# WoodOxen/tactics2d

Hardware: NVIDIA H100
Metric: participant_steps_per_sec (higher is better)
Workload: dtype f32

## Files before the change

### tactics2d_b200/csrc/t2d_kernels.cu

```cuda
#include <cuda_runtime.h>
#include <stddef.h>
#include <stdint.h>
#include <stdio.h>
#include <string.h>

#include <algorithm>
#include <atomic>
#include <cmath>
#include <memory>
#include <mutex>
#include <string>
#include <vector>

#include "../../include/t2d_b200.h"
#include "t2d_math.cuh"

namespace t2d {

constexpr int MAX_WARPS_PER_CTA = 8;
constexpr int CTA_THREADS = MAX_WARPS_PER_CTA * 32;
constexpr int PPL = 4;
constexpr int POSE_PER_WARP = 32 * PPL;
constexpr int MAP_SMEM_LIMIT = 120 * 1024;

struct MapHeader {
  int32_t n_seg, gx, gy, n_items;
  float x0, y0, inv_cell, cell;
  uint32_t off_seg, off_cell, off_items, total_bytes;
  uint32_t off_clear;
  int32_t fine;
  uint32_t off_dcell, off_ditems;
  float dil;
  int32_t n_ditems;
  uint32_t off_objfirst;
  int32_t n_poly;
  uint32_t off_poly;
  uint32_t off_pbox;
  uint32_t off_fine;
  uint32_t smem_bytes;
  float bxmin, bxmax, bymin, bymax;
  int32_t has_bounds;
  uint32_t pad[3];
};
constexpr float CLEAR_QUANT = 0.125f;
static_assert(sizeof(MapHeader) == 128, "MapHeader must be 128 bytes");

struct WorldArgs {
  float *x, *y, *h, *v, *vx, *vy;
  const uint8_t* type_id;
  int32_t* step_count;
  const Params* table;
  int n_types, N, M;
};

struct MapArgs {
  const unsigned char* map_blob;
  const uint32_t* tile_off;
  const uint16_t* tile_id;
};

__device__ __forceinline__ const unsigned char* tile_blob(const MapArgs& m, long long n) {
  return m.map_blob ? m.map_blob + (m.tile_id ? m.tile_off[m.tile_id[n]] : 0u) : nullptr;
}

struct GoalArgs {
  const float* target;
  float* iou;
  float* last_pose;
  int32_t* noact_count;
  float threshold;
  int noact_max;
};

struct StepArgs {
  float *x, *y, *h, *v, *vx, *vy;
  const uint8_t* type_id;
  int32_t* step_count;
  const float* action;
  const float* ego_action;
  uint8_t* flags;
  int16_t* hit_index;
  int16_t* hit_segment;
  uint8_t* scn_status;
  uint8_t* done;
  const unsigned char* map_blob;
  const uint32_t* tile_off;
  const uint16_t* tile_id;
  MapHeader mh;
  const Params* table;
  int map_bytes, map_in_smem;
  int n_types;
  int N, M, G;
  int g_shift, mp_shift, unused1, n_tiles, wpc, table_bytes;
  int off_poseA, off_poseB, off_hit, off_queue, off_sorted, unused0, off_qcount, off_bar;
  int n_steps;
  float dt, dt_rem;
  double dt_d, dt_rem_d, interval_d;
  int max_step, cfg_flags;
  int do_physics, has_bounds, vec_ok, needs_vel_in;
  int prefetch;
  float bxmin, bxmax, bymin, bymax;
  float rb_max;
  GoalArgs goal;
  float *wheel_f, *wheel_r;
};

__device__ __forceinline__ uint32_t smem_u32(const void* p) { return (uint32_t)__cvta_generic_to_shared(p); }

__device__ __forceinline__ void mbar_init(uint64_t* bar, uint32_t count) {
  asm volatile("mbarrier.init.shared::cta.b64 [%0], %1;" ::"r"(smem_u32(bar)), "r"(count));
}
__device__ __forceinline__ void fence_mbar_init() { asm volatile("fence.mbarrier_init.release.cluster;" ::: "memory"); }
__device__ __forceinline__ void mbar_expect_tx(uint64_t* bar, uint32_t bytes) {
  asm volatile("mbarrier.arrive.expect_tx.shared::cta.b64 _, [%0], %1;" ::"r"(smem_u32(bar)), "r"(bytes) : "memory");
}
__device__ __forceinline__ void bulk_g2s(void* dst, const void* src, uint32_t bytes, uint64_t* bar) {
  asm volatile("cp.async.bulk.shared::cluster.global.mbarrier::complete_tx::bytes [%0], [%1], %2, [%3];" ::"r"(
                   smem_u32(dst)),
               "l"(src), "r"(bytes), "r"(smem_u32(bar))
               : "memory");
}
__device__ __forceinline__ void mbar_wait(uint64_t* bar, uint32_t parity) {
  uint32_t ok = 0;
  while (!ok) {
    asm volatile(
        "{\n\t.reg .pred p;\n\t"
        "mbarrier.try_wait.parity.shared::cta.b64 p, [%1], %2;\n\t"
        "selp.u32 %0, 1, 0, p;\n\t}"
        : "=r"(ok)
        : "r"(smem_u32(bar)), "r"(parity)
        : "memory");
  }
}

template <int BYTES> struct VecOf;
template <> struct VecOf<1> { using T = uint8_t; };
template <> struct VecOf<2> { using T = uint16_t; };
template <> struct VecOf<4> { using T = uint32_t; };
template <> struct VecOf<8> { using T = uint2; };
template <> struct VecOf<16> { using T = uint4; };

template <typename T, int N>
__device__ __forceinline__ void ld_vec(const T* p, T (&o)[N]) {
  using V = typename VecOf<sizeof(T) * N>::T;
  const V v = *reinterpret_cast<const V*>(p);
  memcpy(o, &v, sizeof(V));
}
template <typename T, int N>
__device__ __forceinline__ void st_vec(T* p, const T (&o)[N]) {
  using V = typename VecOf<sizeof(T) * N>::T;
  V v;
  memcpy(&v, o, sizeof(V));
  *reinterpret_cast<V*>(p) = v;
}

struct Pose {
  float x, y, h, c, s, l, w;
};

__device__ __noinline__ bool pair_exact(const Pose a, const Pose b) {
  const bool ca = a.w < 0.0f, cb = b.w < 0.0f;
  if (!ca && !cb) return obb_obb_f64(a.x, a.y, a.h, a.l, a.w, b.x, b.y, b.h, b.l, b.w);
  if (!ca && cb) return obb_circle_f64(a.x, a.y, a.h, a.l, a.w, b.x, b.y, b.l);
  if (ca && !cb) return obb_circle_f64(b.x, b.y, b.h, b.l, b.w, a.x, a.y, a.l);
  return circle_circle_f64(a.x, a.y, a.l, b.x, b.y, b.l);
}

__device__ __forceinline__ bool pair_hit(const Pose& a, const Pose& b) {
  const bool ca = a.w < 0.0f, cb = b.w < 0.0f;
  int r;
  if (!ca && !cb) r = obb_obb_f32(a.x, a.y, a.c, a.s, a.l, a.w, b.x, b.y, b.c, b.s, b.l, b.w);
  else if (!ca && cb) r = obb_circle_f32(a.x, a.y, a.c, a.s, a.l, a.w, b.x, b.y, b.l);
  else if (ca && !cb) r = obb_circle_f32(b.x, b.y, b.c, b.s, b.l, b.w, a.x, a.y, a.l);
  else r = circle_circle_f32(a.x, a.y, a.l, b.x, b.y, b.l);
  if (r < 0) return pair_exact(a, b);
  return r != 0;
}

__device__ __noinline__ bool seg_exact(const Pose a, const float4 sg) {
  if (a.w < 0.0f) return circle_segment_f64(a.x, a.y, a.l, sg.x, sg.y, sg.z, sg.w);
  return obb_segment_f64(a.x, a.y, a.h, a.l, a.w, sg.x, sg.y, sg.z, sg.w);
}

__device__ __forceinline__ bool seg_hit(const Pose& a, const float4 sg) {
  int r = a.w < 0.0f ? circle_segment_f32(a.x, a.y, a.l, sg.x, sg.y, sg.z, sg.w)
                     : obb_segment_f32(a.x, a.y, a.c, a.s, a.l, a.w, sg.x, sg.y, sg.z, sg.w);
  if (r < 0) return seg_exact(a, sg);
// ... 409 lines not shown
    if (nvalid == PPL && K1_SHAPE(vec_ok, 1)) {
      ld_vec<float, PPL>(A.x + idx0, sx);
      ld_vec<float, PPL>(A.y + idx0, sy);
      ld_vec<float, PPL>(A.h + idx0, shd);
      ld_vec<float, PPL>(A.v + idx0, sv);
      uint8_t tb8[PPL];
      ld_vec<uint8_t, PPL>(A.type_id + idx0, tb8);
#pragma unroll
      for (int i = 0; i < PPL; ++i) tidv[i] = tb8[i];
      if (K1_SHAPE(do_physics, 1)) {
        float2 act[PPL];
        float lo[4], hi[4];
        ld_vec<float, 4>(A.action + 2 * idx0, lo);
        ld_vec<float, 4>(A.action + 2 * idx0 + 4, hi);
        act[0] = make_float2(lo[0], lo[1]); act[1] = make_float2(lo[2], lo[3]);
        act[2] = make_float2(hi[0], hi[1]); act[3] = make_float2(hi[2], hi[3]);
#pragma unroll
        for (int i = 0; i < PPL; ++i) { a0[i] = act[i].x; a1[i] = act[i].y; }
        if (K1_SHAPE(needs_vel_in, 0)) {
          ld_vec<float, PPL>(A.vx + idx0, svx);
          ld_vec<float, PPL>(A.vy + idx0, svy);
        }
      }
    } else {
#pragma unroll
      for (int i = 0; i < PPL; ++i) {
        if (i < nvalid) {
          sx[i] = A.x[idx0 + i]; sy[i] = A.y[idx0 + i]; shd[i] = A.h[idx0 + i]; sv[i] = A.v[idx0 + i];
          tidv[i] = A.type_id[idx0 + i];
          if (K1_SHAPE(do_physics, 1)) {
            a0[i] = A.action[2 * (idx0 + i)]; a1[i] = A.action[2 * (idx0 + i) + 1];
            if (K1_SHAPE(needs_vel_in, 0)) { svx[i] = A.vx[idx0 + i]; svy[i] = A.vy[idx0 + i]; }
          }
        }
      }
    }
    if (cohorts && !cohort_b && tile == tile0) cohort_arrive(wpc * 32);
    {
      const long long n_next = n + (long long)gridDim.x * wpc * spw;
      if (A.prefetch && n_next < A.N && m0 < M) prefetch_tile_l2<FIXED>(A, n_next * M + m0);
    }
    if (K1_SHAPE(ego_action, nullptr) != nullptr && K1_SHAPE(do_physics, 1) && gl == 0 && scn_ok) {
      const float2 ea = reinterpret_cast<const float2*>(K1_SHAPE(ego_action, nullptr))[n];
      a0[0] = ea.x; a1[0] = ea.y;
    }
    if (!staged) {
      mbar_wait(s_bar, 0);
      staged = true;
    }
    float ch[PPL], sh[PPL];
    bool active[PPL], kin[PPL];
    const Params* pp[PPL];
    int model[PPL];
    bool lane_all_kin = true, lane_any_kin = false;
#pragma unroll
    for (int i = 0; i < PPL; ++i) {
      active[i] = tidv[i] < A.n_types;
      pp[i] = &s_table[active[i] ? tidv[i] : 0];
      model[i] = pp[i]->model_shape & 0xff;
      kin[i] = active[i] && (model[i] == MODEL_KINEMATICS);
      lane_all_kin = lane_all_kin && kin[i];
      lane_any_kin = lane_any_kin || kin[i];
      ch[i] = 1.0f; sh[i] = 0.0f;
    }
    T2D_TL(2, tl_on, tl_slot, sx[PPL - 1] + sy[PPL - 1] + shd[PPL - 1] + sv[PPL - 1] + a0[PPL - 1] + a1[PPL - 1] + (float)model[PPL - 1]);
    if (A.cfg_flags & T2D_CFG_STEER_FIRST) {
#pragma unroll
      for (int i = 0; i < PPL; ++i)
        if (model[i] <= MODEL_DYNAMICS || model[i] == MODEL_DRIFT) { float t = a0[i]; a0[i] = a1[i]; a1[i] = t; }
    }

    if (K1_SHAPE(do_physics, 1)) {
      if (__any_sync(0xffffffffu, lane_any_kin)) {
        const Params* const null_row = &s_table[A.n_types];
        const Params* pk[PPL];
        KinIO<PPL> io;
#pragma unroll
        for (int i = 0; i < PPL; ++i) {
          pk[i] = kin[i] ? pp[i] : null_row;
          io.x[i] = kin[i] ? sx[i] : 0.0f; io.y[i] = kin[i] ? sy[i] : 0.0f;
          io.h[i] = kin[i] ? shd[i] : 0.0f; io.v[i] = kin[i] ? sv[i] : 0.0f;
          io.acc[i] = kin[i] ? a0[i] : 0.0f; io.steer[i] = kin[i] ? a1[i] : 0.0f;
        }
        kinematics_step<PPL>(io, pk, A.n_steps, A.dt, A.dt_rem);
#pragma unroll
        for (int i = 0; i < PPL; ++i) {
          if (kin[i]) {
            sx[i] = io.x[i]; sy[i] = io.y[i]; shd[i] = io.h[i]; sv[i] = io.v[i];
            svx[i] = io.vx[i]; svy[i] = io.vy[i]; ch[i] = io.ch[i]; sh[i] = io.sh[i];
          }
        }
      }
      if (!lane_all_kin) {
#pragma unroll
        for (int i = 0; i < PPL; ++i) {
          if (active[i] && !kin[i]) {
            if constexpr (!KIN_ONLY) {
              OneIO io;
              io.x = sx[i]; io.y = sy[i]; io.h = shd[i]; io.v = sv[i]; io.vx = svx[i]; io.vy = svy[i];
              io.a0 = a0[i]; io.a1 = a1[i];
              io.ch = 1.0f; io.sh = 0.0f;
              other_model_step(io, *pp[i], A.n_steps, A.dt_d, A.dt_rem_d, A.interval_d);
              sx[i] = io.x; sy[i] = io.y; shd[i] = io.h; sv[i] = io.v; svx[i] = io.vx; svy[i] = io.vy;
              ch[i] = io.ch; sh[i] = io.sh;
            } else {
              sincos_fast(shd[i], &sh[i], &ch[i]);
            }
          }
        }
      }
      bool all_active = true;
#pragma unroll
      for (int i = 0; i < PPL; ++i) all_active = all_active && active[i];
      if (nvalid == PPL && K1_SHAPE(vec_ok, 1) && all_active) {
        st_vec<float, PPL>(A.x + idx0, sx);
        st_vec<float, PPL>(A.y + idx0, sy);
        st_vec<float, PPL>(A.h + idx0, shd);
        st_vec<float, PPL>(A.v + idx0, sv);
        st_vec<float, PPL>(A.vx + idx0, svx);
        st_vec<float, PPL>(A.vy + idx0, svy);
      } else {
#pragma unroll
        for (int i = 0; i < PPL; ++i) {
          if (i < nvalid && active[i]) {
            A.x[idx0 + i] = sx[i]; A.y[idx0 + i] = sy[i]; A.h[idx0 + i] = shd[i]; A.v[idx0 + i] = sv[i];
            A.vx[idx0 + i] = svx[i]; A.vy[idx0 + i] = svy[i];
          }
        }
      }
    } else {
#pragma unroll
      for (int i = 0; i < PPL; ++i) sincos_fast(shd[i], &sh[i], &ch[i]);
    }
    T2D_TL(3, tl_on, tl_slot, sx[0] + sy[PPL - 1] + ch[0] + sh[PPL - 1]);

    float px[PPL], py[PPL], rb[PPL];
    unsigned solid_bits = 0;
#pragma unroll
    for (int i = 0; i < PPL; ++i) {
      const Vec4 g2 = params_group(pp[i], 2);
      const bool sol = active[i] && (__float_as_int(g2.w) >> 8) != SHAPE_NONE;
      solid_bits |= sol ? (1u << i) : 0u;
      rb[i] = g2.z;
      px[i] = sol ? sx[i] : __int_as_float(0x7fc00000);
      py[i] = sy[i];
      poseA[i * 32 + lane] = make_float4(px[i], py[i], rb[i], shd[i]);
      poseB[i * 32 + lane] = make_float4(ch[i], sh[i], g2.x, g2.y);
    }
    if (lane == 0) *qcount = 0;
    __syncwarp();
    const int cnt_in = (K1_SHAPE(do_physics, 1) && gl == 0 && scn_ok) ? A.step_count[n] : 0;

    unsigned near_q[PPL], near_alt[PPL];
#pragma unroll
    for (int i = 0; i < PPL; ++i) { near_q[i] = 255u; near_alt[i] = 255u; }
    const MapHeader* lane_mh = &A.mh;
    const unsigned char* lane_blob = A.map_blob;
    if constexpr (MAP_TABLE) {
      lane_blob = A.map_blob + A.tile_off[scn_ok ? A.tile_id[n] : 0];
      lane_mh = reinterpret_cast<const MapHeader*>(lane_blob);
    }
    if (A.map_blob != nullptr && lane_mh->n_seg > 0) {
#pragma unroll
      for (int i = 0; i < PPL; ++i) {
        unsigned alt;
        near_q[i] = near_fetch(px[i], py[i], rb[i], *lane_mh, lane_blob + lane_mh->off_fine, alt);
        near_alt[i] = ((solid_bits >> i) & 1u) ? alt : 255u;
// ... 667 lines not shown
  const long long total = (long long)A.N * A.M;
  for (long long i = (long long)blockIdx.x * blockDim.x + threadIdx.x; i < total; i += (long long)gridDim.x * blockDim.x) {
    const int n = (int)(i / A.M), m = (int)(i - (long long)n * A.M);
    int row;
    if (A.mask != nullptr) {
      if (!A.mask[n]) continue;
      row = A.pool_index ? A.pool_index[n] : n;
      row = min(max(row, 0), A.n_rows - 1);
      if (m == 0) A.log_row_out[n] = row;
    } else {
      row = min(max(A.log_row[n], 0), A.n_rows - 1);
    }
    const long long s = (long long)row * A.M + m;
    int k;
    long long t;
    if (A.slot_track1 != nullptr) {
      k = __ldg(A.slot_track1 + s);
      if (k < 0) {
        if (A.track_out) A.track_out[i] = -1;
        continue;
      }
      t = (long long)A.t0[row] + ((long long)A.step_count[n] + A.offset) * A.interval_ms;
    } else {
      int lo = __ldg(A.slot_off + s), hi = __ldg(A.slot_off + s + 1) - 1;
      if (hi < lo) {
        if (A.track_out) A.track_out[i] = -1;
        continue;
      }
      t = (long long)A.t0[row] + ((long long)A.step_count[n] + A.offset) * A.interval_ms;
      while (lo < hi) {
        const int mid = (lo + hi) >> 1;
        if ((long long)__ldg(&A.entries[mid].last_ms) >= t) hi = mid;
        else lo = mid + 1;
      }
      k = __ldg(&A.entries[lo].track);
    }
    const int4 tr4 = __ldg(reinterpret_cast<const int4*>(A.tracks) + k);
    const int first = tr4.x, period = tr4.y, n_frames = tr4.z, rec_off = tr4.w;
    const long long d = t - first;
    if (d < 0 || d > (long long)(n_frames - 1) * period) {
      A.type_id[i] = T2D_TYPE_INACTIVE;
      if (A.track_out) A.track_out[i] = -1;
      continue;
    }
    if (A.track_out) A.track_out[i] = k;
    const long long j = d / period;
    const int r = (int)(d - j * period);
    const float* a = A.rec + 5 * ((long long)rec_off + j);
    float x, y, h, vx, vy;
    if (r == 0) {
      x = a[0]; y = a[1]; h = a[2]; vx = a[3]; vy = a[4];
    } else {
      const float* b = a + 5;
      const double w = __ddiv_rn((double)r, (double)period);
      x = replay_lerp(a[0], b[0], w);
      y = replay_lerp(a[1], b[1], w);
      vx = replay_lerp(a[3], b[3], w);
      vy = replay_lerp(a[4], b[4], w);
      const double ha = (double)a[2];
      double dh = __dsub_rn((double)b[2], ha);
      if (dh > PI_D) dh = __dsub_rn(dh, TWO_PI_D);
      else if (dh < -PI_D) dh = __dadd_rn(dh, TWO_PI_D);
      double hh = __dadd_rn(ha, __dmul_rn(w, dh));
      if (hh < 0.0) hh = __dadd_rn(hh, TWO_PI_D);
      else if (hh >= TWO_PI_D) hh = __dsub_rn(hh, TWO_PI_D);
      h = __double2float_rn(hh);
      if (h == (float)TWO_PI_D) h = 0.0f;
    }
    const float v = __double2float_rn(__dsqrt_rn(__dadd_rn(__dmul_rn((double)vx, (double)vx), __dmul_rn((double)vy, (double)vy))));
    A.x[i] = x; A.y[i] = y; A.h[i] = h; A.v[i] = v; A.vx[i] = vx; A.vy[i] = vy;
    A.type_id[i] = A.track_type[k];
  }
}

struct PhysArgs {
  Params p;
  float *x, *y, *h, *v, *vx, *vy;
  float *wheel_f, *wheel_r;
  const float* action;
  float* applied;
  int n, n_steps;
  float dt, dt_rem;
  double dt_d, dt_rem_d, interval_d;
};

__global__ void __launch_bounds__(256) t2d_physics_kernel(const __grid_constant__ PhysArgs A) {
  for (long long i = (long long)blockIdx.x * blockDim.x + threadIdx.x; i < A.n; i += (long long)gridDim.x * blockDim.x) {
    if (A.p.model() == MODEL_KINEMATICS) {
      KinIO<1> io;
      io.x[0] = A.x[i]; io.y[0] = A.y[i]; io.h[0] = A.h[i]; io.v[0] = A.v[i];
      io.acc[0] = A.action[2 * i]; io.steer[0] = A.action[2 * i + 1];
      const Params* const p1[1] = {&A.p};
      kinematics_step<1>(io, p1, A.n_steps, A.dt, A.dt_rem);
      A.x[i] = io.x[0]; A.y[i] = io.y[0]; A.h[i] = io.h[0]; A.v[i] = io.v[0]; A.vx[i] = io.vx[0]; A.vy[i] = io.vy[0];
      if (A.applied) { A.applied[2 * i] = io.acc[0]; A.applied[2 * i + 1] = io.steer[0]; }
    } else {
      OneIO io;
      io.x = A.x[i]; io.y = A.y[i]; io.h = A.h[i]; io.v = A.v[i]; io.vx = A.vx[i]; io.vy = A.vy[i];
      io.a0 = A.action[2 * i]; io.a1 = A.action[2 * i + 1];
      io.ch = 1.0f; io.sh = 0.0f;
      if (A.p.model() == MODEL_DRIFT) {
        io.w0 = A.wheel_f[i]; io.w1 = A.wheel_r[i];
        drift_step(io, A.p, A.n_steps, A.dt_d, A.dt_rem_d);
        A.wheel_f[i] = io.w0; A.wheel_r[i] = io.w1;
      } else {
        other_model_step(io, A.p, A.n_steps, A.dt_d, A.dt_rem_d, A.interval_d);
      }
      A.x[i] = io.x; A.y[i] = io.y; A.h[i] = io.h; A.v[i] = io.v; A.vx[i] = io.vx; A.vy[i] = io.vy;
      if (A.applied) { A.applied[2 * i] = io.a0; A.applied[2 * i + 1] = io.a1; }
    }
  }
}

constexpr int LIDAR_EDGES = 144;
constexpr int LIDAR_WARPS = 4;
constexpr int LIDAR_BEAMS = 512;

struct LidarArgs : WorldArgs {
  MapArgs map;
  const double* beam_cs;
  const int16_t* observers;
  float* scan;
  int Q, n_beams;
  double range;
};

__device__ __forceinline__ double point_segment_dist2(double x1, double y1, double x2, double y2) {
  const double dx = x2 - x1, dy = y2 - y1, dd = dx * dx + dy * dy;
  double t = dd > 0.0 ? -(x1 * dx + y1 * dy) / dd : 0.0;
  t = fmin(fmax(t, 0.0), 1.0);
  const double ex = x1 + t * dx, ey = y1 + t * dy;
  return ex * ex + ey * ey;
}

__global__ void __launch_bounds__(LIDAR_WARPS * 32, 7) t2d_lidar_kernel(const __grid_constant__ LidarArgs A) {
  __shared__ double s_edge[LIDAR_WARPS][LIDAR_EDGES][4];
  __shared__ BeamWindow s_win[LIDAR_WARPS][LIDAR_EDGES];
  __shared__ float s_best[LIDAR_WARPS][LIDAR_BEAMS];
  __shared__ int s_cnt[LIDAR_WARPS];
  const int lane = threadIdx.x & 31, warp = threadIdx.x >> 5;
  const long long row = (long long)blockIdx.x * LIDAR_WARPS + warp;
  if (row >= (long long)A.N * A.Q) return;
  const long long n = A.Q == 1 ? row : row <= 0xffffffffll ? (long long)((unsigned)row / (unsigned)A.Q) : row / A.Q;
  const int q = (int)(row - n * A.Q);
  const int jo = A.observers ? (int)A.observers[row] : q;
  double(*edge)[4] = s_edge[warp];
  BeamWindow* win = s_win[warp];
  float* best = s_best[warp];
  int* cnt = &s_cnt[warp];
  const long long base = n * A.M;
  float* out = A.scan + row * A.n_beams;
  if (jo < 0 || jo >= A.M || A.type_id[base + jo] >= A.n_types) {
    for (int b = lane; b < A.n_beams; b += 32) out[b] = INFINITY;
    return;
  }
  const double x0 = A.x[base + jo], y0 = A.y[base + jo], th = A.h[base + jo];
  double sa, ca;
  sincos(th, &sa, &ca);
  const double xoff = -x0 * ca - y0 * sa, yoff = x0 * sa - y0 * ca;
  const double R = A.range, R2 = R * R;
  const unsigned char* blob = tile_blob(A.map, n);
  const MapHeader* tmh = reinterpret_cast<const MapHeader*>(blob);
  const int n_seg = blob ? tmh->n_seg : 0;
  const float4* seg = n_seg > 0 ? reinterpret_cast<const float4*>(blob + tmh->off_seg) : nullptr;
  const int part_rounds = (A.M - 1 + 31) / 32, seg_rounds = (n_seg + 31) / 32;
  for (int b0 = 0; b0 < A.n_beams; b0 += LIDAR_BEAMS) {
    const int nb = min(LIDAR_BEAMS, A.n_beams - b0);
    for (int k = lane; k < nb; k += 32) best[k] = INFINITY;
    if (lane == 0) *cnt = 0;
    __syncwarp();
    for (int r = 0; r < part_rounds + seg_rounds; ++r) {
      if (r < part_rounds) {
        const int i = r * 32 + lane;
        const int j = i < jo ? i : i + 1;
        const int tj = j < A.M ? (int)A.type_id[base + j] : 255;
        if (tj < A.n_types && A.table[tj].shape() == SHAPE_OBB) {
// ... 540 lines not shown
  const uint8_t* ctrl_id = nullptr;
  const int16_t* ctrl_lead = nullptr;
  const int16_t* ctrl_path = nullptr;
  float* ctrl_last_accel = nullptr;
  bool ctrl_has_pid = false;
  bool ctrl_pid_reads_target = false;
  const float* pid_target = nullptr;
  double* pid_state = nullptr;
  dev_ptr<PathVertex> d_path_v;
  dev_ptr<int> d_path_off;
  int n_paths = 0;
  const int16_t* route_id = nullptr;
  double route_threshold = 0.0, route_weight = 0.0;
  float route_off_reward = 0.0f;
  double* route_s_best = nullptr;
  double* route_agent_s_best = nullptr;
  int route_agent_rows = 0;
  std::unique_ptr<ChunkedUpload> hs_upload;
  Mirror hs_out;
  MappedEgo hs_ego;
  AgentStaging ha;
  dev_ptr<uint8_t> ha_flags;
  int host_chunks = 0;
  int n_bev_styles = 0;
  t2d_bev_style bev_style[bev::MAX_STYLES] = {};
  uint8_t bev_type_style[T2D_MAX_TYPES] = {};
  int bev_target_style = bev::NO_STYLE;
  std::unique_ptr<DeviceLog> log;
  std::vector<int> type_model;
};

enum : unsigned { NEED_STATE = 1, NEED_TABLE = 2, NEED_TICK = 4 };

static int require(const t2d_ctx* c, unsigned need) {
  if ((need & NEED_STATE) && !c->x) return fail(T2D_E_STATE, "state not bound: call t2d_bind_state first");
  if ((need & NEED_TABLE) && (!c->d_table || c->n_types == 0))
    return fail(T2D_E_STATE, "type table not set: call t2d_set_type_table first");
  if (need & NEED_TICK) {
    if (c->has_drift && !(c->wheel_f && c->wheel_r))
      return fail(T2D_E_STATE, "the type table holds a SingleTrackDrift row: call t2d_bind_wheel_state first");
    if (c->log && c->log->type_id != c->type_id) return fail(T2D_E_STATE, "state rebound after t2d_set_log: call t2d_set_log again");
  }
  return T2D_OK;
}

static WorldArgs world_args(const t2d_ctx* c) {
  return {c->x, c->y, c->h, c->v, c->vx, c->vy, c->type_id, c->step_count, c->d_table.get(), c->n_types, c->N, c->M};
}

static RouteArgs route_args(const t2d_ctx* c) {
  return {c->route_id, c->d_path_v.get(), c->d_path_off.get(), c->n_paths, c->route_off_reward, c->route_threshold,
          c->route_weight};
}

static int check_route_trackers(const t2d_ctx* c, const char* fn) {
  if (c->route_id && c->route_agent_s_best && c->route_agent_rows != c->agent_q)
    return fail(T2D_E_STATE, std::string(fn) + ": the agents' route tracker has another row count than the bound agents: "
                                               "call t2d_bind_route_trackers again");
  return T2D_OK;
}

static MapArgs map_args(const DeviceMap& map, int first = 0) {
  return {map.blob.get(), map.tile_off.get(), map.tile_id ? map.tile_id + first : nullptr};
}

static int launched() {
  g_launches.fetch_add(1);
  CUDA_TRY(cudaGetLastError());
  return T2D_OK;
}

static int capped_grid(long long items, int per_cta, int sm_count, int per_sm) {
  return (int)std::max(1LL, std::min((items + per_cta - 1) / per_cta, (long long)sm_count * per_sm));
}

template <class Args> static void set_time_step(Args& A, int interval_ms, int delta_t_ms) {
  const int delta_t = std::min(delta_t_ms, interval_ms);
  A.n_steps = interval_ms / delta_t;
  A.dt = (float)((double)delta_t / 1000.0);
  A.dt_rem = (float)((double)(interval_ms % delta_t) / 1000.0);
  A.dt_d = (double)delta_t / 1000.0;
  A.dt_rem_d = (double)(interval_ms % delta_t) / 1000.0;
  A.interval_d = (double)interval_ms / 1000.0;
}

extern "C" {

int t2d_version(void) { return T2D_VERSION; }
const char* t2d_last_error(void) { return g_err.c_str(); }
int64_t t2d_launch_count(void) { return (int64_t)g_launches.load(); }
int64_t t2d_tick_fixed_count(void) { return (int64_t)(g_tick_instances[4].load() + g_tick_instances[5].load()); }
int64_t t2d_tick_instance_count(int k) { return k >= 0 && k < 7 ? (int64_t)g_tick_instances[k].load() : -1; }

#ifdef T2D_TICK_TIMELINE
int t2d_tick_timeline(void* dst, int64_t bytes, int clear) {
  if (!dst || bytes != (int64_t)sizeof(t2d_timeline)) return fail(T2D_E_INVALID, "timeline buffer size");
  CUDA_TRY(cudaMemcpyFromSymbol(dst, t2d_timeline, sizeof(t2d_timeline)));
  if (clear) {
    void* p = nullptr;
    CUDA_TRY(cudaGetSymbolAddress(&p, t2d_timeline));
    CUDA_TRY(cudaMemset(p, 0, sizeof(t2d_timeline)));
  }
  return T2D_OK;
}
#endif

static int check_cfg(const t2d_config* cfg) {
  if (!cfg) return fail(T2D_E_INVALID, "cfg is NULL");
  if (cfg->interval_ms <= 0) return fail(T2D_E_INVALID, "interval_ms must be > 0");
  if (cfg->delta_t_ms <= 0) return fail(T2D_E_INVALID, "delta_t_ms must be > 0");
  return T2D_OK;
}

int t2d_create(t2d_ctx** out, int device, int n_scenarios, int m_participants, const t2d_config* cfg) {
  if (!out) return fail(T2D_E_INVALID, "out is NULL");
  *out = nullptr;
  if (int r = check_cfg(cfg)) return r;
  if (n_scenarios <= 0 || m_participants <= 0) return fail(T2D_E_INVALID, "n_scenarios and m_participants must be > 0");
  if (m_participants > T2D_MAX_PARTICIPANTS)
    return fail(T2D_E_UNSUPPORTED, "m_participants > 128: a scenario must fit one warp (4 participants per lane)");
  int count = 0;
  CUDA_TRY(cudaGetDeviceCount(&count));
  if (device < 0 || device >= count) return fail(T2D_E_INVALID, "no such CUDA device");
  CUDA_TRY(cudaSetDevice(device));
  t2d_ctx* c = new t2d_ctx();
  c->device = device;
  c->N = n_scenarios;
  c->M = m_participants;
  if (const char* e = getenv("T2D_PDL")) c->use_pdl = atoi(e) != 0;
  if (const char* e = getenv("T2D_GRID_LIMIT")) c->grid_limit = std::max(0, atoi(e));
  if (const char* e = getenv("T2D_TICK_GENERIC")) c->tick_generic = atoi(e) != 0;
  if (const char* e = getenv("T2D_PREFETCH")) c->prefetch_override = atoi(e) != 0 ? 1 : 0;
  if (const char* e = getenv("T2D_WPC")) {
    const int v = atoi(e);
    if (v >= 1 && v <= MAX_WARPS_PER_CTA) c->wpc_override = v;
  }
  if (const char* e = getenv("T2D_HOST_CHUNKS")) c->host_chunks = std::max(0, std::min(atoi(e), MAX_HOST_CHUNKS));
  int g = 1;
  while (g * PPL < m_participants) g <<= 1;
  c->G = g;
  c->cfg = *cfg;
  cudaDeviceProp prop;
  CUDA_TRY(cudaGetDeviceProperties(&prop, device));
  c->sm_count = prop.multiProcessorCount;
  c->max_smem_optin = (int)prop.sharedMemPerBlockOptin;
  *out = c;
  return T2D_OK;
}

int t2d_destroy(t2d_ctx* c) {
  if (!c) return T2D_OK;
  cudaSetDevice(c->device);
  delete c;
  return T2D_OK;
}

int t2d_set_config(t2d_ctx* c, const t2d_config* cfg) {
  if (!c) return fail(T2D_E_INVALID, "ctx is NULL");
  if (int r = check_cfg(cfg)) return r;
  c->cfg = *cfg;
  return T2D_OK;
}

int t2d_set_type_table(t2d_ctx* c, const t2d_type_params* table, int n_types) {
  if (!c || !table) return fail(T2D_E_INVALID, "ctx/table is NULL");
  if (n_types <= 0 || n_types > T2D_MAX_TYPES) return fail(T2D_E_INVALID, "n_types must be in 1..64");
// ... 1303 lines not shown
```

### tactics2d_b200/csrc/t2d_math.cuh

```cuda
#pragma once

#include <math.h>
#include <string.h>
#include <stdint.h>

#if defined(__CUDACC__)
#define T2D_HD __host__ __device__ __forceinline__
#define T2D_HD_NOINLINE __host__ __device__ __noinline__
#else
#define T2D_HD inline
#define T2D_HD_NOINLINE
#endif

#if defined(__CUDA_ARCH__)
#define T2D_RSQRTF(x) rsqrtf(x)
#else
#define T2D_RSQRTF(x) (1.0f / sqrtf(x))
#endif

namespace t2d {

constexpr int MODEL_KINEMATICS = 0;
constexpr int MODEL_DYNAMICS = 1;
constexpr int MODEL_POINTMASS_NEWTON = 2;
// ... 67 lines not shown
#endif
}

#if defined(__CUDA_ARCH__)
#define T2D_FDIV(a, b) __fdividef((a), (b))
#else
#define T2D_FDIV(a, b) ((a) / (b))
#endif

constexpr float RINT_MAGIC = 12582912.0f;

T2D_HD float wrap_two_pi(float phi) {
  const float q = (fmaf(phi, INV_TWO_PI, -0.5f) + RINT_MAGIC) - RINT_MAGIC;
  float r = fmaf(-q, TWO_PI_HI, phi);
  r = fmaf(-q, TWO_PI_LO, r);
  if (r < 0.0f) r += TWO_PI_HI;
  if (r >= TWO_PI_HI) r -= TWO_PI_HI;
  if (r < 0.0f) r = 0.0f;
  return r;
}

struct SinCos { float s, c; };
#if defined(__CUDACC__)
__host__ __device__ __noinline__ SinCos sincosf_slow(float x) { SinCos r; sincosf(x, &r.s, &r.c); return r; }
#else
inline SinCos sincosf_slow(float x) { SinCos r; sincosf(x, &r.s, &r.c); return r; }
#endif

T2D_HD void sincos_poly(float r, float& s, float& c) {
  const float z = r * r;
  s = fmaf(r * z, fmaf(z, fmaf(z, -1.9515295891e-4f, 8.3321608736e-3f), -1.6666654611e-1f), r);
  c = fmaf(z * z, fmaf(z, fmaf(z, 2.443315711809948e-5f, -1.388731625493765e-3f), 4.166664568298827e-2f),
           fmaf(-0.5f, z, 1.0f));
}

T2D_HD void sincos_core(float x, float& so, float& co) {
  const float t = fmaf(x, 0.636619772f, RINT_MAGIC);
  const float k = t - RINT_MAGIC;
  float r = fmaf(-k, 1.570556640625f, x);
  r = fmaf(-k, 2.396702766418457e-4f, r);
  r = fmaf(-k, 1.5893254712295857e-8f, r);
  float s, c;
  sincos_poly(r, s, c);
  const int q = float_bits(t);
  const float a = (q & 1) ? c : s, b = (q & 1) ? s : c;
  so = (q & 2) ? -a : a;
  co = ((q + 1) & 2) ? -b : b;
}

T2D_HD void sincos_fast(float x, float* sn, float* cs) {
  float so, co;
  if (!(fabsf(x) <= 512.0f)) {
    const SinCos r = sincosf_slow(x);
    so = r.s; co = r.c;
  } else {
    sincos_core(x, so, co);
  }
  *sn = so;
  *cs = co;
}

constexpr float SIN_C3 = -1.6666667e-1f, SIN_C5 = 8.3333333e-3f;
constexpr float COS_C2 = -0.5f, COS_C4 = 4.1666667e-2f, COS_C6 = -1.3888889e-3f;

T2D_HD void rotate_small(float& c, float& s, float d, float nd) {
  const float dd = d * d;
  const float ts = fmaf(dd, fmaf(dd, SIN_C5, SIN_C3), 1.0f);
  const float sn = d * ts, nsn = nd * ts;
  const float nhv = dd * fmaf(dd, fmaf(dd, COS_C6, COS_C4), COS_C2);
  const float cn = fmaf(s, nsn, fmaf(c, nhv, c));
  const float sm = fmaf(c, sn, fmaf(s, nhv, s));
  c = cn;
  s = sm;
}

template <int W>
struct KinIO {
  float x[W], y[W], h[W], v[W];
  float vx[W], vy[W];
  float ch[W], sh[W];
  float acc[W], steer[W];
};

template <int W>
T2D_HD void kinematics_finish(KinIO<W>& io, const Params* const (&p)[W], const float (&c)[W], const float (&s)[W], float (&v)[W],
                              const float (&Sx)[W], const float (&Sy)[W], const float (&Sv)[W], const float (&kdt)[W],
                              const float (&k)[W], const float (&a)[W], const float (&vlo)[W], const float (&vhi)[W], float dt,
                              float dt_rem) {
#pragma unroll
  for (int i = 0; i < W; ++i) {
    float x = fmaf(dt, Sx[i], io.x[i]);
    float y = fmaf(dt, Sy[i], io.y[i]);
    float dphi = kdt[i] * Sv[i];
    if (dt_rem > 0.0f) {
      x = fmaf(dt_rem * v[i], c[i], x);
      y = fmaf(dt_rem * v[i], s[i], y);
      dphi = fmaf(k[i] * dt_rem, v[i], dphi);
      v[i] = clampf(fmaf(a[i], dt_rem, v[i]), vlo[i], vhi[i]);
    }
    float hn = wrap_two_pi(io.h[i] + dphi);
    float sh, ch;
    sincos_core(hn, sh, ch);
    io.x[i] = x; io.y[i] = y; io.h[i] = hn; io.v[i] = v[i];
    io.vx[i] = v[i] * ch;
    io.vy[i] = v[i] * sh;
    io.ch[i] = ch; io.sh[i] = sh;
  }
}

template <int W>
T2D_HD void kinematics_step(KinIO<W>& io, const Params* const (&p)[W], int n_steps, float dt, float dt_rem) {
  float c[W], s[W], w1[W], Sx[W], Sy[W], Sv[W], kdt[W], adt[W], vlo[W], vhi[W], k[W], a[W];
  bool small = true;
  bool lin = n_steps >= 2 && n_steps <= 24;
  float sd[W], cd[W], sp[W], cp[W];
  bool rare = false;
#pragma unroll
  for (int i = 0; i < W; ++i) {
    const Vec4 g0 = params_group(p[i], 0);
    a[i] = clampf(io.acc[i], g0.x, g0.y);
    const float d = clampf(io.steer[i], g0.z, g0.w);
    io.acc[i] = a[i];
    io.steer[i] = d;
    sincos_poly(d, sd[i], cd[i]);
    sincos_core(io.h[i], sp[i], cp[i]);
    rare = rare || !(fabsf(d) <= 0.78f) || !(fabsf(io.h[i]) <= 512.0f);
  }
  if (rare) {
#pragma unroll
    for (int i = 0; i < W; ++i) {
      if (!(fabsf(io.steer[i]) <= 0.78f)) sincos_fast(io.steer[i], &sd[i], &cd[i]);
      if (!(fabsf(io.h[i]) <= 512.0f)) sincos_fast(io.h[i], &sp[i], &cp[i]);
    }
  }
#pragma unroll
  for (int i = 0; i < W; ++i) {
    const Vec4 g1 = params_group(p[i], 1);
    const float tan_d = T2D_FDIV(sd[i], cd[i]);
    const float tb = g1.z * tan_d;
    const float cb = T2D_RSQRTF(fmaf(tb, tb, 1.0f));
    const float sb = tb * cb;
    k[i] = tan_d * cb * g1.w;
    kdt[i] = k[i] * dt;
    adt[i] = a[i] * dt;
    c[i] = cp[i] * cb - sp[i] * sb;
    s[i] = sp[i] * cb + cp[i] * sb;
    vlo[i] = g1.x;
    vhi[i] = g1.y;
    const float w1u = fmaf(a[i], dt, io.v[i]);
    w1[i] = clampf(w1u, vlo[i], vhi[i]);
    const float wlu = fmaf((float)(n_steps - 1), adt[i], w1[i]);
    const float wl = clampf(fmaf((float)(n_steps - 2), adt[i], w1[i]), vlo[i], vhi[i]);
    lin = lin && (w1u == w1[i]) && (wlu >= vlo[i]) && (wlu <= vhi[i]) && (fabsf(kdt[i] * adt[i]) <= 1e-4f);
    const float wmax = fmaxf(fabsf(io.v[i]), fmaxf(fabsf(w1[i]), fabsf(wl)));
    small = small && (fabsf(kdt[i]) * wmax <= 0.25f);
    Sx[i] = 0.0f; Sy[i] = 0.0f; Sv[i] = 0.0f;
  }
#if defined(__CUDA_ARCH__)
  const bool fast = __all_sync(__activemask(), lin && small);
#else
  const bool fast = lin && small;
#endif
  if (fast) {
    float h[W], nsn[W], se[W], nse[W], he[W];
#pragma unroll
    for (int i = 0; i < W; ++i) {
      const float d0 = kdt[i] * io.v[i], dd = d0 * d0;
      const float ts = fmaf(dd, fmaf(dd, SIN_C5, SIN_C3), 1.0f);
      nsn[i] = (-d0) * ts;
      h[i] = dd * fmaf(dd, fmaf(dd, COS_C6, COS_C4), COS_C2);
      se[i] = kdt[i] * adt[i];
      nse[i] = -se[i];
      he[i] = -0.5f * se[i] * se[i];
    }
    float v[W];
#pragma unroll
    for (int i = 0; i < W; ++i) v[i] = io.v[i];
    {
      float fi = -1.0f;
      for (int it = 0; it < n_steps; ++it) {
        fi += 1.0f;
#pragma unroll
        for (int i = 0; i < W; ++i) {
          Sx[i] = fmaf(v[i], c[i], Sx[i]);
          Sy[i] = fmaf(v[i], s[i], Sy[i]);
          const float sn = -nsn[i];
          const float cn = fmaf(s[i], nsn[i], fmaf(c[i], h[i], c[i]));
          const float sm = fmaf(c[i], sn, fmaf(s[i], h[i], s[i]));
          const float hn = fmaf(nsn[i], se[i], h[i] + he[i]);
          const float nn = fmaf(h[i], nse[i], nsn[i] + nse[i]);
          c[i] = cn; s[i] = sm; h[i] = hn; nsn[i] = nn;
          v[i] = fmaf(fi, adt[i], w1[i]);
        }
      }
    }
    const float nm1 = (float)(n_steps - 1), tri = 0.5f * (float)(n_steps - 1) * (float)(n_steps - 2);
#pragma unroll
    for (int i = 0; i < W; ++i) Sv[i] = fmaf(tri, adt[i], fmaf(nm1, w1[i], io.v[i]));
    kinematics_finish<W>(io, p, c, s, v, Sx, Sy, Sv, kdt, k, a, vlo, vhi, dt, dt_rem);
    return;
  }
  float v[W];
#pragma unroll
  for (int i = 0; i < W; ++i) v[i] = io.v[i];
  if (small) {
    float fi = -1.0f;
    for (int it = 0; it < n_steps; ++it) {
      fi += 1.0f;
#pragma unroll
      for (int i = 0; i < W; ++i) {
        Sx[i] = fmaf(v[i], c[i], Sx[i]);
        Sy[i] = fmaf(v[i], s[i], Sy[i]);
        Sv[i] += v[i];
        rotate_small(c[i], s[i], kdt[i] * v[i], -kdt[i] * v[i]);
        v[i] = clampf(fmaf(fi, adt[i], w1[i]), vlo[i], vhi[i]);
      }
    }
  } else {
    float fi = -1.0f;
    for (int it = 0; it < n_steps; ++it) {
      fi += 1.0f;
#pragma unroll
      for (int i = 0; i < W; ++i) {
        Sx[i] = fmaf(v[i], c[i], Sx[i]);
        Sy[i] = fmaf(v[i], s[i], Sy[i]);
        Sv[i] += v[i];
        float sn, cs;
        sincos_fast(kdt[i] * v[i], &sn, &cs);
        const float c2 = c[i] * cs - s[i] * sn;
        const float s2 = s[i] * cs + c[i] * sn;
        c[i] = c2;
        s[i] = s2;
        v[i] = clampf(fmaf(fi, adt[i], w1[i]), vlo[i], vhi[i]);
      }
    }
  }
  kinematics_finish<W>(io, p, c, s, v, Sx, Sy, Sv, kdt, k, a, vlo, vhi, dt, dt_rem);
}

struct OneIO {
  float x, y, h, v, vx, vy;
  float ch, sh;
  float a0, a1;
  float w0, w1;
};

template <int W>
T2D_HD void dynamics_step_n(OneIO* const (&io)[W], const Params* const (&pp)[W], int n_steps, double dt) {
  double x[W], y[W], phi[W], v[W], d_phi[W], beta[W], sn[W], cs[W];
  double accel[W], delta[W], tan_d[W], L[W], vlo[W], vhi[W], d_beta_slow[W], mu[W];
  double k_a[W], k_sum[W], k_dif[W], k_cc[W], lf_cf_f[W], cf_f[W];
#pragma unroll
  for (int i = 0; i < W; ++i) {
    const Params& p = *pp[i];
    const double lf = p.lf, lr = p.lr;
    L[i] = (double)p.lf + (double)p.lr;
    accel[i] = clampd(io[i]->a0, p.accel_lo, p.accel_hi);
    delta[i] = clampd(io[i]->a1, p.steer_lo, p.steer_hi);
    io[i]->a0 = (float)accel[i];
    io[i]->a1 = (float)delta[i];
    const double mass = p.mass, h = p.mass_height, Iz = p.I_z, cf = p.cf, cr = p.cr;
    mu[i] = p.mu;
    const double factor_f = (G_ACC * lr - accel[i] * h) / L[i];
    const double factor_r = (G_ACC * lf + accel[i] * h) / L[i];
    lf_cf_f[i] = lf * cf * factor_f;
    const double lr_cr_r = lr * cr * factor_r;
    const double lf2_cf_f = lf * lf * cf * factor_f, lr2_cr_r = lr * lr * cr * factor_r;
    cf_f[i] = cf * factor_f;
    const double cr_r = cr * factor_r;
    tan_d[i] = tan(delta[i]);
    const double cos_d = cos(delta[i]);
    x[i] = io[i]->x; y[i] = io[i]->y; phi[i] = io[i]->h; v[i] = io[i]->v;
    d_phi[i] = v[i] / L[i] * tan_d[i];
    beta[i] = atan(lr / lf * tan_d[i]);
    vlo[i] = p.speed_lo; vhi[i] = p.speed_hi;
    d_beta_slow[i] = lr / ((1.0 + tan_d[i] * lr / L[i]) * (1.0 + tan_d[i] * lr / L[i])) / L[i] / (cos_d * cos_d) * delta[i];
    k_a[i] = mu[i] * mass / Iz; k_sum[i] = lf2_cf_f + lr2_cr_r; k_dif[i] = lr_cr_r - lf_cf_f[i]; k_cc[i] = cr_r + cf_f[i];
    sincos(phi[i] + beta[i], &sn[i], &cs[i]);
  }
  for (int it = 0; it < n_steps; ++it) {
#pragma unroll
    for (int i = 0; i < W; ++i) {
      const double dx = v[i] * cs[i], dy = v[i] * sn[i];
      const double v_safe = fabs(v[i]) > 1e-6 ? v[i] : (v[i] >= 0.0 ? 1e-6 : -1e-6);
      double d_beta;
      if (fabs(v[i]) >= 0.1) {
        const double inv_v = 1.0 / v_safe;
        const double w = d_phi[i] * inv_v;
        const double dd_phi = k_a[i] * (lf_cf_f[i] * delta[i] + k_dif[i] * beta[i] - k_sum[i] * w);
        d_beta = mu[i] * inv_v * (cf_f[i] * delta[i] - k_cc[i] * beta[i] + k_dif[i] * w) - d_phi[i];
        d_phi[i] += dd_phi * dt;
      } else {
        d_beta = d_beta_slow[i];
        d_phi[i] += v[i] * cos(beta[i]) / L[i] * tan_d[i] * dt;
      }
      x[i] += dx * dt;
      y[i] += dy * dt;
      v[i] += accel[i] * dt;
      const double dphi_step = d_phi[i] * dt, dbeta_step = d_beta * dt;
      phi[i] += dphi_step;
      beta[i] += dbeta_step;
      v[i] = clampd(v[i], vlo[i], vhi[i]);
      const double d = dphi_step + dbeta_step;
      if (fabs(d) <= 0.1) {
        const double dd = d * d;
        const double sd = d * (1.0 + dd * (-1.0 / 6 + dd * (1.0 / 120 + dd * (-1.0 / 5040 + dd * (1.0 / 362880)))));
        const double hd_ = dd * (-0.5 + dd * (1.0 / 24 + dd * (-1.0 / 720 + dd * (1.0 / 40320 + dd * (-1.0 / 3628800)))));
        const double c2 = cs[i] + (cs[i] * hd_ - sn[i] * sd), s2 = sn[i] + (sn[i] * hd_ + cs[i] * sd);
        cs[i] = c2; sn[i] = s2;
      } else {
        sincos(phi[i] + beta[i], &sn[i], &cs[i]);
      }
    }
  }
#pragma unroll
  for (int i = 0; i < W; ++i) {
    double hd = fmod(phi[i], TWO_PI_D);
    if (hd < 0.0) hd += TWO_PI_D;
    float hn = (float)hd;
    if (hn >= TWO_PI_HI) hn = 0.0f;
// ... 411 lines not shown
```

Baseline: 16.99 billion.

## Replace per-substep kinematic rotation loop with closed-form series evaluation

In the linear/small-angle fast path, the n_steps loop that accumulated rotated velocity sums is replaced by a closed-form evaluation. It uses host-precomputed polynomial series coefficients (kin_series) in the turn angle A and steer-rate term E, passed to kernels via the args struct. The goal is to cut the per-substep FMA chain to a fixed-cost polynomial evaluation. It applies only when |A| and |E| are within bounds across the warp, falls back to the old loop otherwise, and grows kernel parameter size while risking small accuracy differences.

```diff
diff --git a/tactics2d_b200/csrc/t2d_kernels.cu b/tactics2d_b200/csrc/t2d_kernels.cu
--- a/tactics2d_b200/csrc/t2d_kernels.cu
+++ b/tactics2d_b200/csrc/t2d_kernels.cu
@@ -103,6 +103,7 @@
   float rb_max;
   GoalArgs goal;
   float *wheel_f, *wheel_r;
+  KinSeries ks;
 };
 
 __device__ __forceinline__ uint32_t smem_u32(const void* p) { return (uint32_t)__cvta_generic_to_shared(p); }
@@ -678,7 +679,7 @@
           io.h[i] = kin[i] ? shd[i] : 0.0f; io.v[i] = kin[i] ? sv[i] : 0.0f;
           io.acc[i] = kin[i] ? a0[i] : 0.0f; io.steer[i] = kin[i] ? a1[i] : 0.0f;
         }
-        kinematics_step<PPL>(io, pk, A.n_steps, A.dt, A.dt_rem);
+        kinematics_step<PPL>(io, pk, A.n_steps, A.dt, A.dt_rem, A.ks);
 #pragma unroll
         for (int i = 0; i < PPL; ++i) {
           if (kin[i]) {
@@ -1512,6 +1513,7 @@
   int n, n_steps;
   float dt, dt_rem;
   double dt_d, dt_rem_d, interval_d;
+  KinSeries ks;
 };
 
 __global__ void __launch_bounds__(256) t2d_physics_kernel(const __grid_constant__ PhysArgs A) {
@@ -1521,7 +1523,7 @@
       io.x[0] = A.x[i]; io.y[0] = A.y[i]; io.h[0] = A.h[i]; io.v[0] = A.v[i];
       io.acc[0] = A.action[2 * i]; io.steer[0] = A.action[2 * i + 1];
       const Params* const p1[1] = {&A.p};
-      kinematics_step<1>(io, p1, A.n_steps, A.dt, A.dt_rem);
+      kinematics_step<1>(io, p1, A.n_steps, A.dt, A.dt_rem, A.ks);
       A.x[i] = io.x[0]; A.y[i] = io.y[0]; A.h[i] = io.h[0]; A.v[i] = io.v[0]; A.vx[i] = io.vx[0]; A.vy[i] = io.vy[0];
       if (A.applied) { A.applied[2 * i] = io.acc[0]; A.applied[2 * i + 1] = io.steer[0]; }
     } else {
@@ -2228,6 +2230,7 @@
   A.dt_d = (double)delta_t / 1000.0;
   A.dt_rem_d = (double)(interval_ms % delta_t) / 1000.0;
   A.interval_d = (double)interval_ms / 1000.0;
+  A.ks = kin_series(A.n_steps);
 }
 
 extern "C" {
diff --git a/tactics2d_b200/csrc/t2d_math.cuh b/tactics2d_b200/csrc/t2d_math.cuh
--- a/tactics2d_b200/csrc/t2d_math.cuh
+++ b/tactics2d_b200/csrc/t2d_math.cuh
@@ -173,6 +173,83 @@
   float acc[W], steer[W];
 };
 
+constexpr float KS_A_MAX = 1.0f, KS_E_MAX = 0.02f;
+constexpr int KS_R = 4, KS_N_MAX = 24;
+T2D_HD constexpr int ks_deg(int r) { return r == 0 ? 11 : r == 1 ? 10 : r == 2 ? 8 : 5; }
+T2D_HD constexpr int ks_even(int r) { return ks_deg(r) / 2 + 1; }
+T2D_HD constexpr int ks_odd(int r) { return (ks_deg(r) + 1) / 2; }
+T2D_HD constexpr int ks_off(int r) {
+  return (r > 0 ? ks_deg(0) + 1 : 0) + (r > 1 ? ks_deg(1) + 1 : 0) + (r > 2 ? ks_deg(2) + 1 : 0) + (r > 3 ? ks_deg(3) + 1 : 0);
+}
+constexpr int KS_PER_P = ks_off(KS_R);
+struct KinSeries {
+  float c[2][KS_PER_P];
+  float un;
+  int n;
+};
+
+inline KinSeries kin_series(int n) {
+  KinSeries ks;
+  memset(&ks, 0, sizeof(ks));
+  if (n < 2 || n > KS_N_MAX) return ks;
+  ks.n = n;
+  ks.un = (float)((double)(n - 1) / n);
+  for (int p = 0; p < 2; ++p) {
+    for (int r = 0; r < KS_R; ++r) {
+      double w[16];
+      for (int m = 0; m <= ks_deg(r); ++m) {
+        double mom = 0.0;
+        for (int i = 0; i < n; ++i) {
+          const double u = (double)i / n, q = (double)i * (i - 1) / ((double)n * n);
+          mom += (p ? (double)i : 1.0) * pow(u, m) * pow(q, r);
+        }
+        double fact = 1.0;
+        for (int k = 2; k <= m; ++k) fact *= k;
+        for (int k = 2; k <= r; ++k) fact *= k;
+        const double wm = ((m / 2) % 2 ? -mom : mom) / fact;
+        const int k = m % 2 ? ks_even(r) + (ks_odd(r) - 1) - (m - 1) / 2 : (ks_even(r) - 1) - m / 2;
+        w[k] = wm;
+      }
+      float* c = ks.c[p] + ks_off(r);
+      for (int k = 0; k < ks_even(r) + ks_odd(r); ++k) {
+        const int lead = k < ks_even(r) ? 0 : ks_even(r);
+        c[k] = (float)(k == lead ? w[k] : w[lead] != 0.0 ? w[k] / w[lead] : 0.0);
+      }
+    }
+  }
+  return ks;
+}
+
+template <int R>
+T2D_HD void ks_poly(const float* c, float A, float B, float& re, float& im) {
+  float ev = B + c[1];
+#pragma unroll
+  for (int k = 2; k < ks_even(R); ++k) ev = fmaf(ev, B, c[k]);
+  const float* co = c + ks_even(R);
+  float od = B + co[1];
+#pragma unroll
+  for (int k = 2; k < ks_odd(R); ++k) od = fmaf(od, B, co[k]);
+  re = ev * c[0];
+  im = (A * co[0]) * od;
+}
+
+template <int R>
+T2D_HD void ks_step(const float* c, float A, float B, float E, float nE, float& fr, float& fi) {
+  float qr, qi;
+  ks_poly<R>(c + ks_off(R), A, B, qr, qi);
+  const float tr = fmaf(nE, fi, qr);
+  fi = fmaf(E, fr, qi);
+  fr = tr;
+}
+
+T2D_HD void ks_eval(const float* c, float A, float B, float E, float nE, float& fr, float& fi) {
+  static_assert(KS_R == 4, "the chain below runs over r = 3 .. 0");
+  ks_poly<3>(c + ks_off(3), A, B, fr, fi);
+  ks_step<2>(c, A, B, E, nE, fr, fi);
+  ks_step<1>(c, A, B, E, nE, fr, fi);
+  ks_step<0>(c, A, B, E, nE, fr, fi);
+}
+
 template <int W>
 T2D_HD void kinematics_finish(KinIO<W>& io, const Params* const (&p)[W], const float (&c)[W], const float (&s)[W], float (&v)[W],
                               const float (&Sx)[W], const float (&Sy)[W], const float (&Sv)[W], const float (&kdt)[W],
@@ -200,7 +277,8 @@
 }
 
 template <int W>
-T2D_HD void kinematics_step(KinIO<W>& io, const Params* const (&p)[W], int n_steps, float dt, float dt_rem) {
+T2D_HD bool kinematics_step(KinIO<W>& io, const Params* const (&p)[W], int n_steps, float dt, float dt_rem,
+                            const KinSeries& ks = KinSeries()) {
   float c[W], s[W], w1[W], Sx[W], Sy[W], Sv[W], kdt[W], adt[W], vlo[W], vhi[W], k[W], a[W];
   bool small = true;
   bool lin = n_steps >= 2 && n_steps <= 24;
@@ -253,43 +331,87 @@
   const bool fast = lin && small;
 #endif
   if (fast) {
-    float h[W], nsn[W], se[W], nse[W], he[W];
+    const float nm1 = (float)(n_steps - 1), tri = 0.5f * (float)(n_steps - 1) * (float)(n_steps - 2);
+    const float fn = (float)n_steps, hn2 = 0.5f * fn * fn;
+    float A[W], E[W];
+    bool cl = ks.n == n_steps;
 #pragma unroll
     for (int i = 0; i < W; ++i) {
-      const float d0 = kdt[i] * io.v[i], dd = d0 * d0;
-      const float ts = fmaf(dd, fmaf(dd, SIN_C5, SIN_C3), 1.0f);
-      nsn[i] = (-d0) * ts;
-      h[i] = dd * fmaf(dd, fmaf(dd, COS_C6, COS_C4), COS_C2);
-      se[i] = kdt[i] * adt[i];
-      nse[i] = -se[i];
-      he[i] = -0.5f * se[i] * se[i];
-    }
+      A[i] = fn * (kdt[i] * io.v[i]);
+      E[i] = hn2 * (kdt[i] * adt[i]);
+      cl = cl && (fabsf(A[i]) <= KS_A_MAX) && (fabsf(E[i]) <= KS_E_MAX);
+    }
+#if defined(__CUDA_ARCH__)
+    const bool closed = __all_sync(__activemask(), cl);
+#else
+    const bool closed = cl;
+#endif
     float v[W];
-#pragma unroll
-    for (int i = 0; i < W; ++i) v[i] = io.v[i];
-    {
-      float fi = -1.0f;
-      for (int it = 0; it < n_steps; ++it) {
-        fi += 1.0f;
+    if (closed) {
+#pragma unroll
+      for (int i = 0; i < W; ++i) {
+        Sv[i] = fmaf(tri, adt[i], fmaf(nm1, w1[i], io.v[i]));
+        v[i] = fmaf(nm1, adt[i], w1[i]);
+      }
+#pragma unroll
+      for (int i = 0; i < W; ++i) {
+        const float B = A[i] * A[i], nE = -E[i];
+        float fr, fi;
+        ks_eval(ks.c[0], A[i], B, E[i], nE, fr, fi);
+        float gr = io.v[i] * fr, gi = io.v[i] * fi;
+        ks_eval(ks.c[1], A[i], B, E[i], nE, fr, fi);
+        gr = fmaf(adt[i], fr, gr);
+        gi = fmaf(adt[i], fi, gi);
+        Sx[i] = fmaf(c[i], gr, -s[i] * gi);
+        Sy[i] = fmaf(s[i], gr, c[i] * gi);
+      }
+      if (dt_rem > 0.0f) {
 #pragma unroll
         for (int i = 0; i < W; ++i) {
-          Sx[i] = fmaf(v[i], c[i], Sx[i]);
-          Sy[i] = fmaf(v[i], s[i], Sy[i]);
-          const float sn = -nsn[i];
-          const float cn = fmaf(s[i], nsn[i], fmaf(c[i], h[i], c[i]));
-          const float sm = fmaf(c[i], sn, fmaf(s[i], h[i], s[i]));
-          const float hn = fmaf(nsn[i], se[i], h[i] + he[i]);
-          const float nn = fmaf(h[i], nse[i], nsn[i] + nse[i]);
-          c[i] = cn; s[i] = sm; h[i] = hn; nsn[i] = nn;
-          v[i] = fmaf(fi, adt[i], w1[i]);
+          float sn, cs;
+          sincos_core(fmaf(E[i], ks.un, A[i]), sn, cs);
+          const float c2 = fmaf(c[i], cs, -s[i] * sn);
+          s[i] = fmaf(s[i], cs, c[i] * sn);
+          c[i] = c2;
         }
       }
-    }
-    const float nm1 = (float)(n_steps - 1), tri = 0.5f * (float)(n_steps - 1) * (float)(n_steps - 2);
-#pragma unroll
-    for (int i = 0; i < W; ++i) Sv[i] = fmaf(tri, adt[i], fmaf(nm1, w1[i], io.v[i]));
+    } else {
+      float h[W], nsn[W], se[W], nse[W], he[W];
+#pragma unroll
+      for (int i = 0; i < W; ++i) {
+        const float d0 = kdt[i] * io.v[i], dd = d0 * d0;
+        const float ts = fmaf(dd, fmaf(dd, SIN_C5, SIN_C3), 1.0f);
+        nsn[i] = (-d0) * ts;
+        h[i] = dd * fmaf(dd, fmaf(dd, COS_C6, COS_C4), COS_C2);
+        se[i] = kdt[i] * adt[i];
+        nse[i] = -se[i];
+        he[i] = -0.5f * se[i] * se[i];
+      }
+#pragma unroll
+      for (int i = 0; i < W; ++i) v[i] = io.v[i];
+      {
+        float fi = -1.0f;
+        for (int it = 0; it < n_steps; ++it) {
+          fi += 1.0f;
+#pragma unroll
+          for (int i = 0; i < W; ++i) {
+            Sx[i] = fmaf(v[i], c[i], Sx[i]);
+            Sy[i] = fmaf(v[i], s[i], Sy[i]);
+            const float sn = -nsn[i];
+            const float cn = fmaf(s[i], nsn[i], fmaf(c[i], h[i], c[i]));
+            const float sm = fmaf(c[i], sn, fmaf(s[i], h[i], s[i]));
+            const float hn = fmaf(nsn[i], se[i], h[i] + he[i]);
+            const float nn = fmaf(h[i], nse[i], nsn[i] + nse[i]);
+            c[i] = cn; s[i] = sm; h[i] = hn; nsn[i] = nn;
+            v[i] = fmaf(fi, adt[i], w1[i]);
+          }
+        }
+      }
+#pragma unroll
+      for (int i = 0; i < W; ++i) Sv[i] = fmaf(tri, adt[i], fmaf(nm1, w1[i], io.v[i]));
+    }
     kinematics_finish<W>(io, p, c, s, v, Sx, Sy, Sv, kdt, k, a, vlo, vhi, dt, dt_rem);
-    return;
+    return closed;
   }
   float v[W];
 #pragma unroll
@@ -327,6 +449,7 @@
     }
   }
   kinematics_finish<W>(io, p, c, s, v, Sx, Sy, Sv, kdt, k, a, vlo, vhi, dt, dt_rem);
+  return false;
 }
 
 struct OneIO {
```

New measurement: 18.48 billion (median of 6 runs). 1.09x the previous value.
